# poyentung/ebsd-vae

Hardware: AMD Instinct MI355X
Metric: EBSD patterns/sec (128x128, fwd+bwd) (higher is better)
Workload: dtype fp32 I/O, f16x3 split MFMA; 1 GPU; c2: VariationalAutoEncoderRawData 128x128, latent 16, batch 256/GPU, fwd+loss+bwd+Adam; global_batch=256, image_size=128, latent_dim=16, parallelism=dp1

## Files before the change

### ebsd-vae_amd/csrc/conv_wgrad.hip

```cpp
#include <utility>

#include "common.h"
#include "../../include/ebsdvae.h"

namespace ev {

constexpr int WG_PT = 128;
constexpr int WG_AS = 48;

struct WgGeom {
  int TH, TW, NI, ntx, nty, tiles, slices, tps, lTW, ltpx;
};

static int wg_tw_pref() {
  static const int v = evh::env_int("EBSDVAE_WG_TW", 16, 8, 32);
  return (v == 8 || v == 32) ? v : 16;
}

static int wg_block_target(int pt) {
  static const int v = evh::env_int("EBSDVAE_WG_BLOCKS", 512, 64, 8192);
  return pt == 64 ? v : 1024;
}

static bool wg_geom(int B, int H, int W, int cin, int cout, WgGeom* g, int pt = WG_PT) {
// ... 14 lines not shown
  g->lTW = __builtin_ctz(g->TW);
  g->ltpx = __builtin_ctz(g->TH * g->TW);
  if ((1 << g->lTW) != g->TW || (1 << g->ltpx) != g->TH * g->TW) return false;
  g->nty = H / g->TH;
  const long imgs = (B + g->NI - 1) / g->NI;
  g->tiles = (int)(imgs * g->ntx * g->nty);
  const int co_t = cout == 1 ? 1 : (cout == 32 || g->TW == 8 ? cout / 32 : cout / 64);
  const int ci_t = cin == 1 ? 1 : (cout == 1 ? 1 : cin / 32);
  if (co_t <= 0 || ci_t <= 0) return false;
  const int want = wg_block_target(pt) / (co_t * ci_t);
  int tps = 4;
  while ((g->tiles + tps - 1) / tps > (want > 1 ? want : 1)) tps *= 2;
  g->tps = tps;
  g->slices = (g->tiles + tps - 1) / tps;
  return true;
}

static bool wg_pipe() {
  static const bool v = evh::env_flag("EBSDVAE_WG_PIPE", true);
  return v;
}
static int wg_pipe_cot(int cout) {
  static const bool wide = evh::env_flag("EBSDVAE_WG_CO128", true);
  return cout == 32 ? 32 : ((wide && cout % 128 == 0) ? 128 : 64);
}
static int wg_pipe_ci64_mode() {
  static const int v = evh::env_int("EBSDVAE_WG_CI64", 1, 0, 1);
  return v;
}
static int wg_pipe_cit(int cin, int cout) {
  if (wg_pipe_ci64_mode() == 0 || cout == 32 || cin % 64) return 32;
  return wg_pipe_cot(cout) == 64 ? 64 : 32;
}
static bool wg_pipe_geom(int B, int H, int W, int cin, int cout, WgGeom* g) {
  if (B <= 0 || H <= 0 || W <= 0 || cin <= 0 || cout <= 0) return false;
  if (H % 8 || W % 8 || cin % 32 || !(cout == 32 || cout % 64 == 0)) return false;
  if (((H / 8) & (H / 8 - 1)) || ((W / 8) & (W / 8 - 1))) return false;
  if (!ev_buf_bytes_ok(4LL * H * W * (cin > cout ? cin : cout) * 4)) return false;
  g->TW = 8; g->TH = 8; g->NI = 1;
  g->ntx = W / 8; g->nty = H / 8;
  g->lTW = 3; g->ltpx = 6;
  g->tiles = (int)((long)B * g->ntx * g->nty);
  const int cot = wg_pipe_cot(cout), cit = wg_pipe_cit(cin, cout);
  const int co_t = cout == 32 ? 1 : cout / cot;
  const bool eight = cot == 128 || cit == 64;
  const int want = wg_block_target(64) / (eight ? 2 : 1) / (co_t * (cin / cit));
  int tps = 4;
  while ((g->tiles + tps - 1) / tps > (want > 1 ? want : 1)) tps *= 2;
  g->tps = tps;
  g->slices = (g->tiles + tps - 1) / tps;
  return true;
}

static dim3 wg_pipe_grid(const WgGeom& g, int cin, int cout) {
  const int nm = (cout == 32 ? 1 : cout / wg_pipe_cot(cout)) * (cin / wg_pipe_cit(cin, cout));
  return dim3(8 * ((g.slices + 7) / 8) * nm);
}

EV_DEVINL void tile_origin(int t, const WgGeom& g, int& b0, int& y0, int& x0) {
  const int per_img = g.ntx * g.nty;
  const int ib = t / per_img, r = t - ib * per_img;
  b0 = ib * g.NI;
  y0 = (r / g.ntx) * g.TH;
  x0 = (r % g.ntx) * g.TW;
}

template <int TW>
struct WgTile {
  static constexpr int TH = TW == 32 ? 4 : 8;
  static constexpr int NI = TW == 8 ? 2 : 1;
  static constexpr int HP = TH + 2, WP = TW + 2;
  static constexpr int HALO = NI * HP * WP;
  static constexpr int IPX = TH * TW;
  static_assert(NI * IPX == WG_PT, "128-pixel tiles");
  static_assert(HALO * 8 <= 7 * 256, "7 halo float4 items per thread");
};

template <int NWCO, int KSPLIT, int MODE, int TW>
__global__ __launch_bounds__(256, 2) void wgrad_kernel(
    const float* __restrict__ src, const float2* __restrict__ sstats,
    const float* __restrict__ gy, float* __restrict__ wpart, float* __restrict__ bpart, int B,
    int H, int W, int Cin, int Cout, WgGeom g) {
  using T = WgTile<TW>;
  constexpr int CO_T = NWCO * 32;
  constexpr int GS = CO_T + 16;
  constexpr int QG = CO_T / 4;
  constexpr int KG = CO_T / 8;
  constexpr int KH = 7;
  constexpr bool NORM = (MODE == ACT_NORM || MODE == ACT_NORM_UP);
  constexpr bool UPS = (MODE == ACT_UP || MODE == ACT_NORM_UP);
  static_assert(NWCO * 2 * KSPLIT == 4, "4 waves per block");
  static_assert(MODE != ACT_NORM_POOL, "pool-fed layers use the materialised activation");
  constexpr int SPR = TW / (4 * KSPLIT);
  constexpr int ROW_UNROLL = 1;
  extern __shared__ __attribute__((aligned(16))) float smem[];
  float* lg = smem;
  float* la = smem + WG_PT * GS;
  const int tid = threadIdx.x, lane = tid & 63, wave = tid >> 6;
  const int wco = wave % NWCO, wci = (wave / NWCO) & 1, wk = wave / (2 * NWCO);
  const int slice = blockIdx.x, co0 = blockIdx.y * CO_T, ci0 = blockIdx.z * 32;
  const int l16 = lane & 15, kq = lane >> 4;
  const int Hs = UPS ? H / 2 : H, Ws = UPS ? W / 2 : W;
  const int qh = tid & 7;
  const int qg = tid % QG;
  const bool do_bias = blockIdx.z == 0;

  f32x4 acc[2][9];
#pragma unroll
  for (int f = 0; f < 2; ++f)
// ... 418 lines not shown
    for (int s = wk; s < KSTEPS; s += KSPLIT) {
      const int px0 = 32 * s + 4 * gq + q, px1 = px0 + 16;
      bf16x8w a[NPC][2];
#pragma unroll
      for (int i = 0; i < NPC; ++i)
#pragma unroll
        for (int f = 0; f < 2; ++f)
          a[i][f] = tr_frag(gimg + i * GY_PIECE + px0 * GSB + acol + f * 32,
                            gimg + i * GY_PIECE + px1 * GSB + acol + f * 32);
      int hp0, hp1;
      {
        const int im0 = px0 / T::IPX, rm0 = px0 % T::IPX;
        const int im1 = px1 / T::IPX, rm1 = px1 % T::IPX;
        hp0 = (im0 * T::HP + rm0 / TW) * T::WP + rm0 % TW;
        hp1 = (im1 * T::HP + rm1 / TW) * T::WP + rm1 % TW;
      }
      bf16x8w b[NPC];
#pragma unroll
      for (int tap = 0; tap < 9; ++tap) {
        const int toff = (tap / 3) * T::WP + tap % 3;
#pragma unroll
        for (int i = 0; i < NPC; ++i)
          b[i] = tr_frag(aimg + i * ACT_PIECE + (hp0 + toff) * WGS_ASB + bcol,
                         aimg + i * ACT_PIECE + (hp1 + toff) * WGS_ASB + bcol);
#pragma unroll
        for (int f = 0; f < 2; ++f) {
          f32x4 c = acc[f][tap];
          if constexpr (NP == 3) {
            c = __builtin_amdgcn_mfma_f32_16x16x32_bf16(a[1][f], b[1], c, 0, 0, 0);
            c = __builtin_amdgcn_mfma_f32_16x16x32_bf16(a[NP - 1][f], b[0], c, 0, 0, 0);
            c = __builtin_amdgcn_mfma_f32_16x16x32_bf16(a[0][f], b[NP - 1], c, 0, 0, 0);
          }
          c = mfma16_piece<NP>(a[1][f], b[0], c);
          c = mfma16_piece<NP>(a[0][f], b[1], c);
          c = mfma16_piece<NP>(a[0][f], b[0], c);
          acc[f][tap] = c;
        }
      }
    }
  }
  __syncthreads();
  wgrad_split_finish<NWCO, KSPLIT, F16>(acc, bs, wsm, wpart, bpart, slice, co0, ci0, Cin, Cout, gsc,
                                        do_bias);
}

template <class F, int... I>
EV_DEVINL void static_for_impl(F&& f, std::integer_sequence<int, I...>) {
  (f(std::integral_constant<int, I>()), ...);
}
template <int N, class F>
EV_DEVINL void static_for(F&& f) {
  static_for_impl(f, std::make_integer_sequence<int, N>());
}

template <int Q>
EV_DEVINL int wg_store_perm(int r) {
  if constexpr (Q == 8) return (r & ~3) | ((r >> 1) & 1) | ((r & 1) << 1);
  return r;
}

template <int NP, int NWCO, int KSPLIT, int MODE, int NWCI = 2, int FCO = 2>
__global__ __launch_bounds__(NWCO * NWCI * KSPLIT * 64, NWCO * NWCI * KSPLIT >= 8 ? 1 : 2) void wgrad_pipe_kernel(
    const float* __restrict__ src, const float2* __restrict__ sstats,
    const float* __restrict__ gy, float* __restrict__ wpart, float* __restrict__ bpart, int B,
    int H, int W, int Cin, int Cout, WgGeom g, const float* __restrict__ gmax, int gmT) {
  constexpr int TW = 8, PT = 64;
  using T = WgTileP<TW, PT>;
  constexpr int NPC = npc(NP);
  constexpr bool F16 = NP == NP_F16;
  constexpr int CO_T = NWCO * 16 * FCO;
  constexpr int CI_T = NWCI * 16;
  constexpr int GSB = CO_T * 2 + 32;
  constexpr int ASB = CI_T * 2 + 32;
  constexpr int QG = CO_T / 4;
  constexpr int QH = CI_T / 4;
  constexpr int NTH = NWCO * NWCI * KSPLIT * 64;
  constexpr int KG = PT * CO_T / 4 / NTH;
  constexpr int KH = (T::HALO * QH + NTH - 1) / NTH;
  constexpr int NIT = KG + KH;
  constexpr int KSTEPS = PT / 32;
  constexpr int NSLOT = (KSTEPS / KSPLIT) * 9;
  constexpr int GY_PIECE = PT * GSB;
  constexpr int ACT_PIECE = T::HALO * ASB;
  constexpr int BUF = NPC * (GY_PIECE + ACT_PIECE);
  constexpr bool NORM = (MODE == ACT_NORM || MODE == ACT_NORM_UP);
  constexpr bool UPS = (MODE == ACT_UP || MODE == ACT_NORM_UP);
  constexpr int kGyPol = CO_T <= 64 ? 2 : 0;
  static_assert(T::NI == 1 && T::HP == 10 && T::WP == 10, "8x8 tiles");
  static_assert(NWCO * NWCI * KSPLIT == 4 || NWCO * NWCI * KSPLIT == 8, "4 or 8 waves per block");
  static_assert((NWCI == 2 || NWCI == 4) && (FCO == 2 || FCO == 4), "wave / block tiles");
  static_assert(NTH % QG == 0 && NTH % QH == 0, "item channel groups fixed per thread");
  static_assert(KSTEPS % KSPLIT == 0 && NIT <= NSLOT, "item slots");
  static_assert(MODE != ACT_NORM_POOL, "pool-fed layers use the materialised activation");
  extern __shared__ __attribute__((aligned(16))) char wsm[];
  const int tid = threadIdx.x, lane = tid & 63, wave = tid >> 6;
  const int wco = wave % NWCO, wci = (wave / NWCO) % NWCI, wk = wave / (NWCI * NWCO);
  const int nco = Cout / CO_T, nm = nco * (Cin / CI_T);
  const int xcd = blockIdx.x & 7, wq = blockIdx.x >> 3, m = wq % nm;
  const int slice = (wq / nm) * 8 + xcd;
  if (slice >= g.slices) return;
  const int co0 = (m % nco) * CO_T, ci0 = (m / nco) * CI_T;
  const int Hs = UPS ? H / 2 : H, Ws = UPS ? W / 2 : W;
  const int qh = tid % QH, qg = tid % QG;

  f32x4 acc[FCO][9];
#pragma unroll
  for (int f = 0; f < FCO; ++f)
#pragma unroll
    for (int t = 0; t < 9; ++t) acc[f][t] = f32x4{0.f, 0.f, 0.f, 0.f};
  double bs[4] = {0.0, 0.0, 0.0, 0.0};

  const int per_img = g.ntx * g.nty;
  const int t_beg = slice * g.tps;
  const int t_end = min(t_beg + g.tps, g.tiles);
  int gshift = 0;
  if constexpr (F16)
    if (t_beg < t_end) gshift = f16_gshift(gmax, gmT, t_beg / per_img, (t_end - 1) / per_img);
  const float gsc = ldexpf(1.f, gshift);

  int gyo[KG], glo[KG];
#pragma unroll
  for (int k = 0; k < KG; ++k) {
    const int px = wg_store_perm<QG>((tid + NTH * k) / QG), r = px / TW, c = px % TW;
    gyo[k] = (r * W + c) * Cout + co0 + qg * 4;
    glo[k] = px * GSB + qg * 8;
  }
  int hdr[KH], hdc[KH], hlo[KH];
  int hbo[KH];
  const int srow = Ws * Cin * 4;
#pragma unroll
  for (int k = 0; k < KH; ++k) {
    const int pix = wg_store_perm<QH>((tid + NTH * k) / QH);
    hdr[k] = pix < T::HALO ? pix / T::WP - 1 : -(1 << 20);
    hdc[k] = pix % T::WP - 1;
    hlo[k] = pix * ASB + qh * 8;
    hbo[k] = pix < T::HALO ? (UPS ? (hdr[k] >> 1) * srow + (hdc[k] >> 1) * Cin * 4
                                  : hdr[k] * srow + hdc[k] * Cin * 4) + (ci0 + qh * 4) * 4
                           : (int)0x80000000;
  }
  const int gimg_bytes = H * W * Cout * 4, simg_bytes = Hs * Ws * Cin * 4;

  float4 rg[KG], rh[KH];
  float2 st_l[4], st_s[4];
  int lb = 0, ly = 0, lx = 0;
  int sb = 0, sy = 0, sx = 0;
  const int lgx = 31 - __builtin_clz(g.ntx), lgp = lgx + 31 - __builtin_clz(g.nty);
  auto tile_at = [&](int t, int& b0, int& y0, int& x0) EV_LAMBDA_INLINE {
    const int rr = t & ((1 << lgp) - 1);
    b0 = t >> lgp; y0 = (rr >> lgx) * T::TH; x0 = (rr & (g.ntx - 1)) * TW;
  };
  __amdgpu_buffer_rsrc_t rgy, rsrc;
  int gtoff = 0, stoff = 0;
  auto set_tile = [&]() EV_LAMBDA_INLINE {
    rgy = __builtin_amdgcn_make_buffer_rsrc((void*)(gy + (size_t)lb * H * W * Cout), 0, gimg_bytes,
                                            0x00020000);
    rsrc = __builtin_amdgcn_make_buffer_rsrc((void*)(src + (size_t)lb * Hs * Ws * Cin), 0,
                                             simg_bytes, 0x00020000);
    gtoff = (ly * W + lx) * Cout * 4;
    stoff = UPS ? (ly >> 1) * srow + (lx >> 1) * Cin * 4 : ly * srow + lx * Cin * 4;
  };
  auto load_stats = [&]() EV_LAMBDA_INLINE {
    set_tile();
    if constexpr (NORM) {
      const float2* sp = sstats + (size_t)lb * Cin + ci0 + qh * 4;
      st_l[0] = norm_fs(sp[0]); st_l[1] = norm_fs(sp[1]); st_l[2] = norm_fs(sp[2]); st_l[3] = norm_fs(sp[3]);
    }
  };
  auto in_img = [&](int k, int y0, int x0) EV_LAMBDA_INLINE {
    return (unsigned)(y0 + hdr[k]) < (unsigned)H && (unsigned)(x0 + hdc[k]) < (unsigned)W;
  };
  auto issue_item = [&](auto j_c) EV_LAMBDA_INLINE {
    constexpr int j = decltype(j_c)::value;
    if constexpr (j < KG) {
      rg[j] = __builtin_bit_cast(float4, __builtin_amdgcn_raw_buffer_load_b128(
                                             rgy, gtoff + gyo[j] * 4, 0, kGyPol));
    } else {
      constexpr int k = j - KG;
      rh[k] = __builtin_bit_cast(float4, __builtin_amdgcn_raw_buffer_load_b128(
                                             rsrc, stoff + hbo[k], 0, 0));
    }
  };
  float4 tb;
  auto store_item = [&](auto j_c, char* buf) EV_LAMBDA_INLINE {
    constexpr int j = decltype(j_c)::value;
    if constexpr (j < KG) {
      float4 v = rg[j];
      tb.x += v.x; tb.y += v.y; tb.z += v.z; tb.w += v.w;
      if constexpr (F16) v = make_float4(v.x * gsc, v.y * gsc, v.z * gsc, v.w * gsc);
      store_pieces<NP>(buf + glo[j], GY_PIECE, v);
    } else {
      constexpr int k = j - KG;
      if (hdr[k] > -2) {
        float4 v = make_float4(0.f, 0.f, 0.f, 0.f);
        if (in_img(k, sy, sx)) {
          v = rh[k];
          if (NORM)
            v = make_float4(normact_fs(v.x, st_s[0]), normact_fs(v.y, st_s[1]),
                            normact_fs(v.z, st_s[2]), normact_fs(v.w, st_s[3]));
        }
        store_pieces<NP>(buf + NPC * GY_PIECE + hlo[k], ACT_PIECE, v);
      }
    }
  };
  auto all_items = [&](auto fn) EV_LAMBDA_INLINE { static_for<NIT>(fn); };
  auto shift = [&]() EV_LAMBDA_INLINE {
    sb = lb; sy = ly; sx = lx;
#pragma unroll
    for (int i = 0; i < 4; ++i) st_s[i] = st_l[i];
  };

  const int gq = lane >> 4, i16 = lane & 15, q = i16 >> 2, p4 = i16 & 3;
  const int acol = (wco * 16 * FCO + 4 * p4) * 2;
  const int bcol = (wci * 16 + 4 * p4) * 2;

  if (t_beg < t_end) {
    tile_at(t_beg, lb, ly, lx);
    load_stats();
    all_items([&](auto j) EV_LAMBDA_INLINE { issue_item(j); });
    shift();
    tb = make_float4(0.f, 0.f, 0.f, 0.f);
    all_items([&](auto j) EV_LAMBDA_INLINE { store_item(j, wsm); });
    bs[0] += (double)tb.x; bs[1] += (double)tb.y; bs[2] += (double)tb.z; bs[3] += (double)tb.w;
    tile_at(min(t_beg + 1, t_end - 1), lb, ly, lx);
    load_stats();
    all_items([&](auto j) EV_LAMBDA_INLINE { issue_item(j); });
  }
  __syncthreads();
  for (int t = t_beg; t < t_end; ++t) {
    const int cur = (t - t_beg) & 1;
    const char* gimg = wsm + cur * BUF;
    const char* aimg = gimg + NPC * GY_PIECE;
    char* nbuf = wsm + (1 - cur) * BUF;
    shift();
    tile_at(min(t + 2, t_end - 1), lb, ly, lx);
    load_stats();
    tb = make_float4(0.f, 0.f, 0.f, 0.f);
    static_for<KSTEPS / KSPLIT>([&](auto si_c) EV_LAMBDA_INLINE {
      constexpr int si = decltype(si_c)::value;
      const int s = wk + si * KSPLIT;
      const int px0 = 32 * s + 4 * gq + q, px1 = px0 + 16;
      bf16x8w a[NPC][FCO];
#pragma unroll
      for (int i = 0; i < NPC; ++i)
#pragma unroll
        for (int f = 0; f < FCO; ++f)
          a[i][f] = tr_frag(gimg + i * GY_PIECE + px0 * GSB + acol + f * 32,
                            gimg + i * GY_PIECE + px1 * GSB + acol + f * 32);
      const int hp0 = (px0 / TW) * T::WP + px0 % TW, hp1 = (px1 / TW) * T::WP + px1 % TW;
      static_for<9>([&](auto tap_c) EV_LAMBDA_INLINE {
        constexpr int tap = decltype(tap_c)::value;
        constexpr int toff = (tap / 3) * T::WP + tap % 3;
        bf16x8w b[NPC];
#pragma unroll
        for (int i = 0; i < NPC; ++i)
          b[i] = tr_frag(aimg + i * ACT_PIECE + (hp0 + toff) * ASB + bcol,
                         aimg + i * ACT_PIECE + (hp1 + toff) * ASB + bcol);
#pragma unroll
        for (int f = 0; f < FCO; ++f) {
          f32x4 c = acc[f][tap];
          c = mfma16_piece<NP>(a[1][f], b[0], c);
          c = mfma16_piece<NP>(a[0][f], b[1], c);
          c = mfma16_piece<NP>(a[0][f], b[0], c);
          acc[f][tap] = c;
        }
        all_items([&](auto j_c) EV_LAMBDA_INLINE {
          constexpr int j = decltype(j_c)::value;
          if constexpr (si * 9 + tap == (j * NSLOT) / NIT) {
            store_item(j_c, nbuf);
            issue_item(j_c);
          }
        });
      });
    });
    if (t + 1 < t_end) {
      bs[0] += (double)tb.x; bs[1] += (double)tb.y; bs[2] += (double)tb.z; bs[3] += (double)tb.w;
    }
    __syncthreads();
  }
  wgrad_split_finish<NWCO, KSPLIT, F16, FCO, NWCI>(acc, bs, wsm, wpart, bpart, slice, co0, ci0, Cin,
                                                   Cout, gsc, ci0 == 0);
}

__global__ __launch_bounds__(128) void wgrad_cin1_kernel(
    const float* __restrict__ src, const float2* __restrict__ sstats, int smode,
    const float* __restrict__ gy, float* __restrict__ wpart, float* __restrict__ bpart, int B,
    int H, int W, int Cout, WgGeom g) {
  constexpr int GS = 48;
  extern __shared__ __attribute__((aligned(16))) float smem[];
  float* lg = smem;
  float* la = smem + WG_PT * GS;
  const int tid = threadIdx.x, lane = tid & 63, wave = tid >> 6;
  const int slice = blockIdx.x;
  const int HP = g.TH + 2, WP = g.TW + 2, halo = g.NI * HP * WP;
  const int l16 = lane & 15, kq = lane >> 4;
  const int tapj = l16 < 9 ? l16 : 0;
  const int tkh = tapj / 3, tkw = tapj % 3;
  f32x4 acc = f32x4{0.f, 0.f, 0.f, 0.f};
  double bsum = 0.0;
  const int t_beg = slice * g.tps, t_end = min(t_beg + g.tps, g.tiles);
  const int tpx = g.TH * g.TW;
  for (int t = t_beg; t < t_end; ++t) {
    int b0, y0, x0;
    tile_origin(t, g, b0, y0, x0);
    __syncthreads();
    for (int i = tid; i < WG_PT * 8; i += 128) {
      const int px = i >> 3, q = i & 7;
      const int img = px >> g.ltpx, rem = px & (tpx - 1);
      const int r = rem >> g.lTW, c = rem & (g.TW - 1);
      const int gb = b0 + img;
// ... 229 lines not shown
    once = true;
  }
  hipLaunchKernelGGL(k, grid, dim3(256), lds, s, src, (const float2*)st, gy, wpart, bpart, B, H, W,
                     cin, cout, g);
}

template <int NWCO, int KSPLIT, int MODE>
static void launch_wg(dim3 grid, size_t lds, hipStream_t s, const float* src, const float* st,
                      const float* gy, float* wpart, float* bpart, int B, int H, int W, int cin,
                      int cout, const WgGeom& g) {
  if (g.TW == 32)
    launch_wg_tw<NWCO, KSPLIT, MODE, 32>(grid, lds, s, src, st, gy, wpart, bpart, B, H, W, cin, cout, g);
  else if (g.TW == 16)
    launch_wg_tw<NWCO, KSPLIT, MODE, 16>(grid, lds, s, src, st, gy, wpart, bpart, B, H, W, cin, cout, g);
  else if constexpr (NWCO == 1)
    launch_wg_tw<NWCO, KSPLIT, MODE, 8>(grid, lds, s, src, st, gy, wpart, bpart, B, H, W, cin, cout, g);
}

template <int NP, int NWCO, int KSPLIT, int MODE, int TW, int PT>
static void launch_wgs_tw(dim3 grid, hipStream_t s, const float* src, const float* st,
                          const float* gy, float* wpart, float* bpart, int B, int H, int W, int cin,
                          int cout, const WgGeom& g, const float* gmax, int gmT) {
  using T = WgTileP<TW, PT>;
  constexpr int CO_T = NWCO * 32;
  const size_t lds_img = (size_t)npc(NP) * ((size_t)PT * (CO_T * 2 + 32) + (size_t)T::HALO * WGS_ASB);
  const size_t lds_fold = KSPLIT == 2 ? (size_t)2 * 72 * 64 * 4 : 0;
  const size_t lds_bias = 256 * 4 * 8;
  size_t lds = lds_img;
  if (lds < lds_fold) lds = lds_fold;
  if (lds < lds_bias) lds = lds_bias;
  auto k = wgrad_split_kernel<NP, NWCO, KSPLIT, MODE, TW, PT>;
  static bool once = false;
  if (!once) {
    (void)hipFuncSetAttribute((const void*)k, hipFuncAttributeMaxDynamicSharedMemorySize, 160 * 1024);
    once = true;
  }
  hipLaunchKernelGGL(k, grid, dim3(256), lds, s, src, (const float2*)st, gy, wpart, bpart, B, H, W,
                     cin, cout, g, gmax, gmT);
}

template <int NP, int NWCO, int KSPLIT, int MODE>
static void launch_wgs(dim3 grid, hipStream_t s, const float* src, const float* st, const float* gy,
                       float* wpart, float* bpart, int B, int H, int W, int cin, int cout,
                       const WgGeom& g, const float* gmax, int gmT) {
  constexpr int PT = 64;
  if (g.TW == 32)
    launch_wgs_tw<NP, NWCO, KSPLIT, MODE, 32, PT>(grid, s, src, st, gy, wpart, bpart, B, H, W, cin, cout, g, gmax, gmT);
  else if (g.TW == 16)
    launch_wgs_tw<NP, NWCO, KSPLIT, MODE, 16, PT>(grid, s, src, st, gy, wpart, bpart, B, H, W, cin, cout, g, gmax, gmT);
  else if constexpr (NWCO == 1)
    launch_wgs_tw<NP, NWCO, KSPLIT, MODE, 8, PT>(grid, s, src, st, gy, wpart, bpart, B, H, W, cin, cout, g, gmax, gmT);
}

template <int NP, int NWCO, int KSPLIT, int MODE, int NWCI = 2, int FCO = 2>
static void launch_wgp(dim3 grid, hipStream_t s, const float* src, const float* st, const float* gy,
                       float* wpart, float* bpart, int B, int H, int W, int cin, int cout,
                       const WgGeom& g, const float* gmax, int gmT) {
  constexpr int CO_T = NWCO * 16 * FCO, CI_T = NWCI * 16;
  constexpr int NTH = NWCO * NWCI * KSPLIT * 64;
  const size_t lds_img = 2 * (size_t)npc(NP) * ((size_t)64 * (CO_T * 2 + 32) + (size_t)100 * (CI_T * 2 + 32));
  const size_t lds_fold = KSPLIT == 2 ? (size_t)NWCO * NWCI * FCO * 36 * 64 * 4 : 0;
  size_t lds = lds_img;
  if (lds < lds_fold) lds = lds_fold;
  if (lds < (size_t)NTH * 4 * 8) lds = (size_t)NTH * 4 * 8;
  auto k = wgrad_pipe_kernel<NP, NWCO, KSPLIT, MODE, NWCI, FCO>;
  static bool once = false;
  if (!once) {
    (void)hipFuncSetAttribute((const void*)k, hipFuncAttributeMaxDynamicSharedMemorySize, 160 * 1024);
    once = true;
  }
  hipLaunchKernelGGL(k, grid, dim3(NTH), lds, s, src, (const float2*)st, gy, wpart, bpart, B, H, W,
                     cin, cout, g, gmax, gmT);
}

template <class F>
static void with_src_mode(int mode, F&& f) {
  evh::with_const<ACT_RAW, ACT_NORM, ACT_UP, ACT_NORM_UP>(mode, f);
}
template <int N> using Int = std::integral_constant<int, N>;

template <int NP>
static void dispatch_wgp(int mode, bool narrow, dim3 grid, hipStream_t s, const float* src,
                         const float* st, const float* gy, float* wpart, float* bpart, int B, int H,
                         int W, int cin, int cout, const WgGeom& g, const float* gmax, int gmT) {
  with_src_mode(mode, [&](auto m) {
    auto go = [&](auto nwco, auto ksplit, auto nwci) {
      launch_wgp<NP, decltype(nwco)::value, decltype(ksplit)::value, decltype(m)::value,
                 decltype(nwci)::value>(grid, s, src, st, gy, wpart, bpart, B, H, W, cin, cout, g, gmax, gmT);
    };
    if (narrow) go(Int<1>(), Int<2>(), Int<2>());
    else if (wg_pipe_cit(cin, cout) == 64) go(Int<2>(), Int<1>(), Int<4>());
    else if (wg_pipe_cot(cout) == 128) go(Int<4>(), Int<1>(), Int<2>());
    else go(Int<2>(), Int<1>(), Int<2>());
  });
}

template <int NP>
static void dispatch_wgs(int mode, bool narrow, dim3 grid, hipStream_t s, const float* src,
                         const float* st, const float* gy, float* wpart, float* bpart, int B, int H,
                         int W, int cin, int cout, const WgGeom& g, const float* gmax, int gmT) {
  with_src_mode(mode, [&](auto m) {
    constexpr int M = decltype(m)::value;
    if (narrow) launch_wgs<NP, 1, 2, M>(grid, s, src, st, gy, wpart, bpart, B, H, W, cin, cout, g, gmax, gmT);
    else launch_wgs<NP, 2, 1, M>(grid, s, src, st, gy, wpart, bpart, B, H, W, cin, cout, g, gmax, gmT);
  });
}

static bool wgs_geom_ok(const WgGeom& g, int pt) {
  if (pt == 128)
    return (g.TW == 32 && g.TH == 4) || (g.TW == 16 && g.TH == 8 && g.NI == 1) ||
           (g.TW == 8 && g.TH == 8 && g.NI == 2);
  return (g.TW == 32 && g.TH == 2) || (g.TW == 16 && g.TH == 4 && g.NI == 1) ||
         (g.TW == 8 && g.TH == 8 && g.NI == 1);
}

}

using namespace ev;

extern "C" int ebsdvae_conv3x3_wgrad_split_slices(int B, int H, int W, int cin, int cout, int pieces) {
  WgGeom g;
  if (pieces != 2 && pieces != 3 && pieces != NP_F16) return -1;
  if (B <= 0 || H <= 0 || W <= 0 || cin <= 0 || cout <= 0) return -1;
  if (cin % 32 || !(cout == 32 || cout % 64 == 0)) return -1;
  if (pieces != 3 && wg_pipe()) return wg_pipe_geom(B, H, W, cin, cout, &g) ? g.slices : -1;
  const int pt = 64;
  if (!wg_geom(B, H, W, cin, cout, &g, pt) || !wgs_geom_ok(g, pt)) return -1;
  return g.slices;
}

extern "C" int ebsdvae_conv3x3_wgrad_split(const float* src, const float* src_stats, int src_mode,
                                           const float* gy, float* wpart, float* bpart, int B,
                                           int H, int W, int cin, int cout, int pieces,
                                           ebsdvae_stream_t stream) {
  WgGeom g;
  EV_REQUIRE(src && gy && wpart && bpart && B > 0, "conv3x3_wgrad_split: null pointer");
  EV_REQUIRE(pieces == 2 || pieces == 3, "conv3x3_wgrad_split: pieces=%d (2 or 3)", pieces);
  EV_REQUIRE(src_mode >= 0 && src_mode <= 4 && src_mode != ACT_NORM_POOL,
             "conv3x3_wgrad_split: bad src_mode %d (pool-fed layers pass the pooled activation RAW)",
             src_mode);
  EV_REQUIRE(src_mode == ACT_RAW || src_mode == ACT_UP || src_stats, "conv3x3_wgrad_split: NORM needs stats");
  EV_REQUIRE(cin % 32 == 0 && (cout == 32 || cout % 64 == 0), "conv3x3_wgrad_split: cin=%d cout=%d unsupported",
             cin, cout);
  hipStream_t s = (hipStream_t)stream;
  if (pieces == 2 && wg_pipe()) {
    EV_REQUIRE(wg_pipe_geom(B, H, W, cin, cout, &g), "conv3x3_wgrad_split: unsupported shape H=%d W=%d", H, W);
    const bool narrow = cout == 32;
    dispatch_wgp<2>(src_mode, narrow, wg_pipe_grid(g, cin, cout), s, src, src_stats, gy, wpart, bpart, B,
                    H, W, cin, cout, g, nullptr, 0);
    return evh::check_launch("wgrad_split");
  }
  const int pt = 64;
  EV_REQUIRE(wg_geom(B, H, W, cin, cout, &g, pt) && wgs_geom_ok(g, pt),
             "conv3x3_wgrad_split: unsupported shape H=%d W=%d", H, W);
  const bool narrow = cout == 32 || g.TW == 8 || (pieces == 3 && g.TW == 16);
  const dim3 grid(g.slices, narrow ? cout / 32 : cout / 64, cin / 32);
  if (pieces == 3)
    dispatch_wgs<3>(src_mode, narrow, grid, s, src, src_stats, gy, wpart, bpart, B, H, W, cin, cout, g,
                    nullptr, 0);
  else
    dispatch_wgs<2>(src_mode, narrow, grid, s, src, src_stats, gy, wpart, bpart, B, H, W, cin, cout, g,
                    nullptr, 0);
  return evh::check_launch("wgrad_split");
}

extern "C" int ebsdvae_conv3x3_wgrad_f16(const float* src, const float* src_stats, int src_mode,
                                         const float* gy, const float* gmax, int gm_tiles,
                                         float* wpart, float* bpart, int B, int H, int W, int cin,
                                         int cout, ebsdvae_stream_t stream) {
  WgGeom g;
  EV_REQUIRE(src && gy && gmax && gm_tiles > 0 && wpart && bpart && B > 0,
             "conv3x3_wgrad_f16: null pointer or no gradient maxima");
  EV_REQUIRE(src_mode >= 0 && src_mode <= 4 && src_mode != ACT_NORM_POOL,
             "conv3x3_wgrad_f16: bad src_mode %d (pool-fed layers pass the pooled activation RAW)",
             src_mode);
  EV_REQUIRE(src_mode == ACT_RAW || src_mode == ACT_UP || src_stats, "conv3x3_wgrad_f16: NORM needs stats");
  EV_REQUIRE(cin % 32 == 0 && (cout == 32 || cout % 64 == 0), "conv3x3_wgrad_f16: cin=%d cout=%d unsupported",
             cin, cout);
  if (wg_pipe()) {
    EV_REQUIRE(wg_pipe_geom(B, H, W, cin, cout, &g), "conv3x3_wgrad_f16: unsupported shape H=%d W=%d", H, W);
    const bool narrow = cout == 32;
    dispatch_wgp<NP_F16>(src_mode, narrow, wg_pipe_grid(g, cin, cout), (hipStream_t)stream, src, src_stats,
                         gy, wpart, bpart, B, H, W, cin, cout, g, gmax, gm_tiles);
    return evh::check_launch("wgrad_f16");
  }
  const int pt = 64;
  EV_REQUIRE(wg_geom(B, H, W, cin, cout, &g, pt) && wgs_geom_ok(g, pt),
             "conv3x3_wgrad_f16: unsupported shape H=%d W=%d", H, W);
  const bool narrow = cout == 32 || g.TW == 8;
  const dim3 grid(g.slices, narrow ? cout / 32 : cout / 64, cin / 32);
  dispatch_wgs<NP_F16>(src_mode, narrow, grid, (hipStream_t)stream, src, src_stats, gy, wpart, bpart,
                       B, H, W, cin, cout, g, gmax, gm_tiles);
  return evh::check_launch("wgrad_f16");
}

extern "C" int ebsdvae_conv3x3_wgrad_slices(int B, int H, int W, int cin, int cout) {
  WgGeom g;
  if (!wg_geom(B, H, W, cin, cout, &g)) return -1;
  return g.slices;
}

extern "C" int ebsdvae_conv3x3_wgrad(const float* src, const float* src_stats, int src_mode,
                                     const float* gy, float* wpart, float* bpart, int B, int H,
                                     int W, int cin, int cout, ebsdvae_stream_t stream) {
  WgGeom g;
  EV_REQUIRE(src && gy && wpart && bpart && B > 0, "conv3x3_wgrad: null pointer");
  EV_REQUIRE(src_mode >= 0 && src_mode <= 4, "conv3x3_wgrad: bad src_mode");
  EV_REQUIRE(src_mode == ACT_RAW || src_mode == ACT_UP || src_stats, "conv3x3_wgrad: NORM needs stats");
  EV_REQUIRE(wg_geom(B, H, W, cin, cout, &g), "conv3x3_wgrad: unsupported shape H=%d W=%d", H, W);
  hipStream_t s = (hipStream_t)stream;
  if (cin == 1) {
    EV_REQUIRE(cout == 32, "conv3x3_wgrad: cin=1 needs cout=32");
    hipLaunchKernelGGL(wgrad_cin1_kernel, dim3(g.slices), dim3(128), wg_lds(1, g, 32), s, src,
                       (const float2*)src_stats, src_mode, gy, wpart, bpart, B, H, W, cout, g);
    return evh::check_launch("wgrad_cin1");
  }
  if (cout == 1) {
    EV_REQUIRE(cin == 32, "conv3x3_wgrad: cout=1 needs cin=32");
    hipLaunchKernelGGL(wgrad_cout1_kernel, dim3(g.slices), dim3(128), wg_lds(2, g, 0), s, src,
                       (const float2*)src_stats, src_mode, gy, wpart, bpart, B, H, W, cin, g);
    return evh::check_launch("wgrad_cout1");
  }
  EV_REQUIRE(cin % 32 == 0 && (cout == 32 || cout % 64 == 0), "conv3x3_wgrad: cin=%d cout=%d unsupported",
             cin, cout);
  EV_REQUIRE((g.TW == 32 && g.TH == 4) || (g.TW == 16 && g.TH == 8 && g.NI == 1) ||
                 (g.TW == 8 && g.TH == 8 && g.NI == 2),
             "conv3x3_wgrad: unsupported tile geometry H=%d W=%d", H, W);
  EV_REQUIRE(src_mode != ACT_NORM_POOL,
             "conv3x3_wgrad: pass the pooled activation materialised by the forward (RAW)");
  const bool narrow = cout == 32 || g.TW == 8;
  const size_t lds = wg_lds(0, g, narrow ? 32 : 64);
  const dim3 grid(g.slices, cout / (narrow ? 32 : 64), cin / 32);
  with_src_mode(src_mode, [&](auto m) {
    constexpr int M = decltype(m)::value;
    if (narrow) launch_wg<1, 2, M>(grid, lds, s, src, src_stats, gy, wpart, bpart, B, H, W, cin, cout, g);
    else launch_wg<2, 1, M>(grid, lds, s, src, src_stats, gy, wpart, bpart, B, H, W, cin, cout, g);
// ... 78 lines not shown
```

Before: 30450 patterns/s.

## Add parity-decomposed and source-resolution-halo wgrad paths for upsample-fed convs

Adds two new variants of the pipelined weight-gradient kernel for layers fed by a nearest-neighbour upsample. The parity path (off by default) splits output pixels into four parity classes so each correlates against the low-resolution source with 2x2 effective taps, then folds them into the 3x3 weights. The source-halo path (on by default) stages only a 6x6 source-resolution halo instead of the 10x10 upsampled one and remaps the tap addresses. Both aim to cut halo loads and LDS traffic, at the cost of more template instances and more complex indexing.

```diff
diff --git a/ebsd-vae_amd/csrc/conv_wgrad.hip b/ebsd-vae_amd/csrc/conv_wgrad.hip
--- a/ebsd-vae_amd/csrc/conv_wgrad.hip
+++ b/ebsd-vae_amd/csrc/conv_wgrad.hip
@@ -90,9 +90,34 @@
   return true;
 }
 
+static bool wg_upphase() {
+  static const bool v = evh::env_flag("EBSDVAE_WG_UPPHASE", false);
+  return v;
+}
+static bool wg_srchalo() {
+  static const bool v = evh::env_flag("EBSDVAE_WG_SRCHALO", true);
+  return v;
+}
+static int wg_upp_shape(int mode, int H, int W, int cin, int cout) {
+  if (!wg_upphase() || !(mode == ACT_UP || mode == ACT_NORM_UP) || H % 16 || W % 16) return 0;
+  if (cout == 32) return 1;
+  return (wg_pipe_ci64_mode() != 0 && cin % 64 == 0 && cout % 64 == 0) ? 2 : 0;
+}
+static bool wg_pipe_geom_upp(int shape, int B, int H, int W, int cin, int cout, WgGeom* g) {
+  if (!shape || H % 16 || W % 16 || !wg_pipe_geom(B, H, W, cin, cout, g)) return false;
+  const int nm = shape == 1 ? cin / 32 : (cout / 64) * (cin / 64);
+  const int want = wg_block_target(64) / (shape == 2 ? 2 : 1) / nm;
+  g->ntx = W / 16; g->nty = H / 16;
+  g->tiles = (int)((long)B * g->ntx * g->nty);
+  int tps = 1;
+  while ((g->tiles + tps - 1) / tps > (want > 1 ? want : 1)) tps *= 2;
+  g->tps = tps;
+  return g->slices == (g->tiles + tps - 1) / tps;
+}
+
+static dim3 wg_pipe_grid(const WgGeom& g, int nm) { return dim3(8 * ((g.slices + 7) / 8) * nm); }
 static dim3 wg_pipe_grid(const WgGeom& g, int cin, int cout) {
-  const int nm = (cout == 32 ? 1 : cout / wg_pipe_cot(cout)) * (cin / wg_pipe_cit(cin, cout));
-  return dim3(8 * ((g.slices + 7) / 8) * nm);
+  return wg_pipe_grid(g, (cout == 32 ? 1 : cout / wg_pipe_cot(cout)) * (cin / wg_pipe_cit(cin, cout)));
 }
 
 EV_DEVINL void tile_origin(int t, const WgGeom& g, int& b0, int& y0, int& x0) {
@@ -617,6 +642,7 @@
 EV_DEVINL void static_for(F&& f) {
   static_for_impl(f, std::make_integer_sequence<int, N>());
 }
+template <int N> using Int = std::integral_constant<int, N>;
 
 template <int Q>
 EV_DEVINL int wg_store_perm(int r) {
@@ -624,7 +650,11 @@
   return r;
 }
 
-template <int NP, int NWCO, int KSPLIT, int MODE, int NWCI = 2, int FCO = 2>
+#ifndef EV_WG_UP_GD
+#define EV_WG_UP_GD 1
+#endif
+template <int NP, int NWCO, int KSPLIT, int MODE, int NWCI = 2, int FCO = 2, bool UPP = false,
+          bool SH = false>
 __global__ __launch_bounds__(NWCO * NWCI * KSPLIT * 64, NWCO * NWCI * KSPLIT >= 8 ? 1 : 2) void wgrad_pipe_kernel(
     const float* __restrict__ src, const float2* __restrict__ sstats,
     const float* __restrict__ gy, float* __restrict__ wpart, float* __restrict__ bpart, int B,
@@ -641,7 +671,9 @@
   constexpr int QH = CI_T / 4;
   constexpr int NTH = NWCO * NWCI * KSPLIT * 64;
   constexpr int KG = PT * CO_T / 4 / NTH;
-  constexpr int KH = (T::HALO * QH + NTH - 1) / NTH;
+  constexpr int HWP = SH ? 6 : T::WP;
+  constexpr int HALO_N = SH ? 36 : T::HALO;
+  constexpr int KH = (HALO_N * QH + NTH - 1) / NTH;
   constexpr int NIT = KG + KH;
   constexpr int KSTEPS = PT / 32;
   constexpr int NSLOT = (KSTEPS / KSPLIT) * 9;
@@ -657,6 +689,8 @@
   static_assert(NTH % QG == 0 && NTH % QH == 0, "item channel groups fixed per thread");
   static_assert(KSTEPS % KSPLIT == 0 && NIT <= NSLOT, "item slots");
   static_assert(MODE != ACT_NORM_POOL, "pool-fed layers use the materialised activation");
+  static_assert(!UPP || (UPS && FCO == 2 && KH <= 4), "parity steps: upsample-fed, 16 x FCO accumulators");
+  static_assert(!SH || (UPS && !UPP), "source-resolution halo: upsample-fed, full-resolution steps");
   extern __shared__ __attribute__((aligned(16))) char wsm[];
   const int tid = threadIdx.x, lane = tid & 63, wave = tid >> 6;
   const int wco = wave % NWCO, wci = (wave / NWCO) % NWCI, wk = wave / (NWCI * NWCO);
@@ -669,10 +703,12 @@
   const int qh = tid % QH, qg = tid % QG;
 
   f32x4 acc[FCO][9];
-#pragma unroll
-  for (int f = 0; f < FCO; ++f)
-#pragma unroll
-    for (int t = 0; t < 9; ++t) acc[f][t] = f32x4{0.f, 0.f, 0.f, 0.f};
+  if constexpr (!UPP) {
+#pragma unroll
+    for (int f = 0; f < FCO; ++f)
+#pragma unroll
+      for (int t = 0; t < 9; ++t) acc[f][t] = f32x4{0.f, 0.f, 0.f, 0.f};
+  }
   double bs[4] = {0.0, 0.0, 0.0, 0.0};
 
   const int per_img = g.ntx * g.nty;
@@ -687,7 +723,7 @@
 #pragma unroll
   for (int k = 0; k < KG; ++k) {
     const int px = wg_store_perm<QG>((tid + NTH * k) / QG), r = px / TW, c = px % TW;
-    gyo[k] = (r * W + c) * Cout + co0 + qg * 4;
+    gyo[k] = (UPP ? 2 * (r * W + c) : r * W + c) * Cout + co0 + qg * 4;
     glo[k] = px * GSB + qg * 8;
   }
   int hdr[KH], hdc[KH], hlo[KH];
@@ -696,10 +732,10 @@
 #pragma unroll
   for (int k = 0; k < KH; ++k) {
     const int pix = wg_store_perm<QH>((tid + NTH * k) / QH);
-    hdr[k] = pix < T::HALO ? pix / T::WP - 1 : -(1 << 20);
-    hdc[k] = pix % T::WP - 1;
+    hdr[k] = pix < HALO_N ? pix / HWP - 1 : -(1 << 20);
+    hdc[k] = pix % HWP - 1;
     hlo[k] = pix * ASB + qh * 8;
-    hbo[k] = pix < T::HALO ? (UPS ? (hdr[k] >> 1) * srow + (hdc[k] >> 1) * Cin * 4
+    hbo[k] = pix < HALO_N ? (UPS && !UPP && !SH ? (hdr[k] >> 1) * srow + (hdc[k] >> 1) * Cin * 4
                                   : hdr[k] * srow + hdc[k] * Cin * 4) + (ci0 + qh * 4) * 4
                            : (int)0x80000000;
   }
@@ -717,12 +753,13 @@
   __amdgpu_buffer_rsrc_t rgy, rsrc;
   int gtoff = 0, stoff = 0;
   auto set_tile = [&]() EV_LAMBDA_INLINE {
-    rgy = __builtin_amdgcn_make_buffer_rsrc((void*)(gy + (size_t)lb * H * W * Cout), 0, gimg_bytes,
-                                            0x00020000);
+    if constexpr (!UPP)
+      rgy = __builtin_amdgcn_make_buffer_rsrc((void*)(gy + (size_t)lb * H * W * Cout), 0, gimg_bytes,
+                                              0x00020000);
     rsrc = __builtin_amdgcn_make_buffer_rsrc((void*)(src + (size_t)lb * Hs * Ws * Cin), 0,
                                              simg_bytes, 0x00020000);
     gtoff = (ly * W + lx) * Cout * 4;
-    stoff = UPS ? (ly >> 1) * srow + (lx >> 1) * Cin * 4 : ly * srow + lx * Cin * 4;
+    stoff = UPS && !UPP ? (ly >> 1) * srow + (lx >> 1) * Cin * 4 : ly * srow + lx * Cin * 4;
   };
   auto load_stats = [&]() EV_LAMBDA_INLINE {
     set_tile();
@@ -732,7 +769,10 @@
     }
   };
   auto in_img = [&](int k, int y0, int x0) EV_LAMBDA_INLINE {
-    return (unsigned)(y0 + hdr[k]) < (unsigned)H && (unsigned)(x0 + hdc[k]) < (unsigned)W;
+    if constexpr (SH)
+      return (unsigned)((y0 >> 1) + hdr[k]) < (unsigned)Hs && (unsigned)((x0 >> 1) + hdc[k]) < (unsigned)Ws;
+    return (unsigned)(y0 + hdr[k]) < (unsigned)(UPP ? Hs : H) &&
+           (unsigned)(x0 + hdc[k]) < (unsigned)(UPP ? Ws : W);
   };
   auto issue_item = [&](auto j_c) EV_LAMBDA_INLINE {
     constexpr int j = decltype(j_c)::value;
@@ -778,6 +818,195 @@
   const int acol = (wco * 16 * FCO + 4 * p4) * 2;
   const int bcol = (wci * 16 + 4 * p4) * 2;
 
+  if constexpr (UPP) {
+    constexpr int GD = EV_WG_UP_GD;
+    static_assert(GD == 1 || GD == 2, "gy prefetch depth");
+    constexpr int NSL = (KSTEPS / KSPLIT) * 4;
+    constexpr int HSTEP = 4 / KH >= 1 ? 4 / KH : 1;
+    static_assert(KG + 1 <= NSL, "item slots of a parity step");
+    f32x4 pacc[FCO][16];
+#pragma unroll
+    for (int f = 0; f < FCO; ++f)
+#pragma unroll
+      for (int t = 0; t < 16; ++t) pacc[f][t] = f32x4{0.f, 0.f, 0.f, 0.f};
+    float4 rq[GD][KG];
+    __amdgpu_buffer_rsrc_t rgy_c, rgy_s;
+    int gt_c = 0, gt_s = 0;
+    int pof[4];
+#pragma unroll
+    for (int par = 0; par < 4; ++par) pof[par] = ((par >> 1) * W + (par & 1)) * Cout * 4;
+    auto gy_tile = [&](int b0, int y0, int x0, __amdgpu_buffer_rsrc_t& r, int& off) EV_LAMBDA_INLINE {
+      r = __builtin_amdgcn_make_buffer_rsrc((void*)(gy + (size_t)b0 * H * W * Cout), 0, gimg_bytes,
+                                            0x00020000);
+      off = (2 * y0 * W + 2 * x0) * Cout * 4;
+    };
+    constexpr int GROWS = NTH / QG / TW;
+    static_assert(GROWS * TW * QG == NTH && (NTH / QG) % 4 == 0, "gy items whole tile rows apart");
+    const int gyv = gyo[0] * 4, glv = glo[0];
+    const int gstep = GROWS * 2 * W * Cout * 4;
+    int hpk[KH];
+#pragma unroll
+    for (int k = 0; k < KH; ++k) {
+      const int pix = wg_store_perm<QH>((tid + NTH * k) / QH);
+      hpk[k] = pix < T::HALO ? ((pix / T::WP) << 16) | (pix % T::WP) : (0x7fff << 16);
+    }
+    const int hcv = (ci0 + qh * 4) * 4;
+    auto issue_gy = [&](auto v_c, auto j_c) EV_LAMBDA_INLINE {
+      constexpr int v = decltype(v_c)::value, j = decltype(j_c)::value;
+      rq[v & (GD - 1)][j] = __builtin_bit_cast(
+          float4, __builtin_amdgcn_raw_buffer_load_b128(v >= 4 ? rgy_s : rgy_c, gyv,
+                                                        (v >= 4 ? gt_s : gt_c) + pof[v & 3] + j * gstep,
+                                                        kGyPol));
+    };
+    auto store_gy = [&](auto v_c, auto j_c, char* buf) EV_LAMBDA_INLINE {
+      constexpr int v = decltype(v_c)::value, j = decltype(j_c)::value;
+      float4 w = rq[v & (GD - 1)][j];
+      tb.x += w.x; tb.y += w.y; tb.z += w.z; tb.w += w.w;
+      if constexpr (F16) w = make_float4(w.x * gsc, w.y * gsc, w.z * gsc, w.w * gsc);
+      store_pieces<NP>(buf + glv + j * (NTH / QG) * GSB, GY_PIECE, w);
+    };
+    auto issue_h = [&](auto k_c) EV_LAMBDA_INLINE {
+      constexpr int k = decltype(k_c)::value;
+      const int hr = (hpk[k] >> 16) - 1, hc = (hpk[k] & 0xffff) - 1;
+      const int vo = hr < T::HP ? stoff + hr * srow + hc * Cin * 4 + hcv : (int)0x80000000;
+      rh[k] = __builtin_bit_cast(float4, __builtin_amdgcn_raw_buffer_load_b128(rsrc, vo, 0, 0));
+    };
+    auto store_h = [&](auto k_c, char* buf) EV_LAMBDA_INLINE {
+      constexpr int k = decltype(k_c)::value;
+      const int hr = hpk[k] >> 16, hc = hpk[k] & 0xffff;
+      if (hr < T::HP) {
+        float4 v = make_float4(0.f, 0.f, 0.f, 0.f);
+        if ((unsigned)(sy + hr - 1) < (unsigned)Hs && (unsigned)(sx + hc - 1) < (unsigned)Ws) {
+          v = rh[k];
+          if (NORM)
+            v = make_float4(normact_fs(v.x, st_s[0]), normact_fs(v.y, st_s[1]),
+                            normact_fs(v.z, st_s[2]), normact_fs(v.w, st_s[3]));
+        }
+        store_pieces<NP>(buf + NPC * GY_PIECE + (hr * T::WP + hc) * ASB + qh * 8, ACT_PIECE, v);
+      }
+    };
+    auto stage_tile = [&]() EV_LAMBDA_INLINE {
+      sb = lb; sy = ly; sx = lx;
+      if constexpr (NORM) {
+        const float2* sp = sstats + (size_t)sb * Cin + ci0 + qh * 4;
+        st_s[0] = norm_fs(sp[0]); st_s[1] = norm_fs(sp[1]); st_s[2] = norm_fs(sp[2]); st_s[3] = norm_fs(sp[3]);
+      }
+    };
+    if (t_beg < t_end) {
+      tile_at(t_beg, lb, ly, lx);
+      set_tile();
+      gy_tile(lb, ly, lx, rgy_s, gt_s);
+      rgy_c = rgy_s; gt_c = gt_s;
+      static_for<KH>([&](auto k) EV_LAMBDA_INLINE { issue_h(k); });
+      static_for<KG>([&](auto j) EV_LAMBDA_INLINE { issue_gy(Int<0>(), j); });
+      stage_tile();
+      tb = make_float4(0.f, 0.f, 0.f, 0.f);
+      static_for<KG>([&](auto j) EV_LAMBDA_INLINE { store_gy(Int<0>(), j, wsm); });
+      static_for<KH>([&](auto k) EV_LAMBDA_INLINE { store_h(k, wsm); });
+      bs[0] += (double)tb.x; bs[1] += (double)tb.y; bs[2] += (double)tb.z; bs[3] += (double)tb.w;
+      tile_at(min(t_beg + 1, t_end - 1), lb, ly, lx);
+      set_tile();
+      static_for<KH>([&](auto k) EV_LAMBDA_INLINE { issue_h(k); });
+      static_for<GD>([&](auto d) EV_LAMBDA_INLINE {
+        static_for<KG>([&](auto j) EV_LAMBDA_INLINE { issue_gy(Int<1 + decltype(d)::value>(), j); });
+      });
+    }
+    __syncthreads();
+    for (int t = t_beg; t < t_end; ++t) {
+      const int aset = (t - t_beg) & 1;
+      const char* aimg = wsm + aset * BUF + NPC * GY_PIECE;
+      char* anext = wsm + (1 - aset) * BUF;
+#pragma unroll
+      for (int k = 0; k < KH; ++k) asm volatile("" : "+v"(hpk[k]));
+      rgy_c = rgy_s; gt_c = gt_s;
+      stage_tile();
+      gy_tile(sb, sy, sx, rgy_s, gt_s);
+      tile_at(min(t + 2, t_end - 1), lb, ly, lx);
+      set_tile();
+      static_for<4>([&](auto par_c) EV_LAMBDA_INLINE {
+        constexpr int par = decltype(par_c)::value, py = par >> 1, px = par & 1;
+        constexpr int hk = par / HSTEP;
+        constexpr bool has_h = par % HSTEP == 0 && hk < KH;
+        constexpr int NITP = KG + (has_h ? 1 : 0);
+        const char* gimg = wsm + (par & 1) * BUF;
+        char* gnext = wsm + ((par + 1) & 1) * BUF;
+        tb = make_float4(0.f, 0.f, 0.f, 0.f);
+        static_for<KSTEPS / KSPLIT>([&](auto si_c) EV_LAMBDA_INLINE {
+          constexpr int si = decltype(si_c)::value;
+          const int s = wk + si * KSPLIT;
+          const int px0 = 32 * s + 4 * gq + q, px1 = px0 + 16;
+          bf16x8w a[NPC][FCO];
+#pragma unroll
+          for (int i = 0; i < NPC; ++i)
+#pragma unroll
+            for (int f = 0; f < FCO; ++f)
+              a[i][f] = tr_frag(gimg + i * GY_PIECE + px0 * GSB + acol + f * 32,
+                                gimg + i * GY_PIECE + px1 * GSB + acol + f * 32);
+          const int hp0 = (px0 / TW) * T::WP + px0 % TW, hp1 = (px1 / TW) * T::WP + px1 % TW;
+          static_for<4>([&](auto tt_c) EV_LAMBDA_INLINE {
+            constexpr int tt = decltype(tt_c)::value;
+            constexpr int toff = (py + (tt >> 1)) * T::WP + px + (tt & 1);
+            bf16x8w b[NPC];
+#pragma unroll
+            for (int i = 0; i < NPC; ++i)
+              b[i] = tr_frag(aimg + i * ACT_PIECE + (hp0 + toff) * ASB + bcol,
+                             aimg + i * ACT_PIECE + (hp1 + toff) * ASB + bcol);
+#pragma unroll
+            for (int f = 0; f < FCO; ++f) {
+              f32x4 c = pacc[f][par * 4 + tt];
+              c = mfma16_piece<NP>(a[1][f], b[0], c);
+              c = mfma16_piece<NP>(a[0][f], b[1], c);
+              c = mfma16_piece<NP>(a[0][f], b[0], c);
+              pacc[f][par * 4 + tt] = c;
+            }
+            static_for<KG>([&](auto j_c) EV_LAMBDA_INLINE {
+              constexpr int j = decltype(j_c)::value;
+              if constexpr (si * 4 + tt == (j * NSL) / NITP) {
+                store_gy(Int<par + 1>(), j_c, gnext);
+                issue_gy(Int<par + 1 + GD>(), j_c);
+              }
+            });
+            if constexpr (has_h && si * 4 + tt == (KG * NSL) / NITP) {
+              store_h(Int<hk>(), anext);
+              issue_h(Int<hk>());
+            }
+          });
+        });
+        if (par < 3 || t + 1 < t_end) {
+          bs[0] += (double)tb.x; bs[1] += (double)tb.y; bs[2] += (double)tb.z; bs[3] += (double)tb.w;
+        }
+        __syncthreads();
+      });
+    }
+#pragma unroll
+    for (int f = 0; f < FCO; ++f)
+#pragma unroll
+      for (int tap = 0; tap < 9; ++tap) {
+        const int ky = tap / 3, kx = tap % 3;
+        f32x4 c = f32x4{0.f, 0.f, 0.f, 0.f};
+#pragma unroll
+        for (int par = 0; par < 4; ++par) {
+          const int py = par >> 1, px = par & 1;
+          const int ay = py == 0 ? (ky >= 1) : (ky == 2), ax = px == 0 ? (kx >= 1) : (kx == 2);
+          c += pacc[f][par * 4 + ay * 2 + ax];
+        }
+        acc[f][tap] = c;
+      }
+    wgrad_split_finish<NWCO, KSPLIT, F16, FCO, NWCI>(acc, bs, wsm, wpart, bpart, slice, co0, ci0, Cin,
+                                                     Cout, gsc, ci0 == 0);
+    return;
+  }
+
+  int sh_ry[3], sh_cx[3];
+  if constexpr (SH) {
+    const int pxw = 32 * wk + 4 * gq + q, r = pxw / TW, c = pxw % TW;
+#pragma unroll
+    for (int d = 0; d < 3; ++d) {
+      sh_ry[d] = (((r + d - 1) >> 1) + 1) * HWP * ASB + bcol;
+      sh_cx[d] = (((c + d - 1) >> 1) + 1) * ASB;
+    }
+  }
+
   if (t_beg < t_end) {
     tile_at(t_beg, lb, ly, lx);
     load_stats();
@@ -816,10 +1045,17 @@
         constexpr int tap = decltype(tap_c)::value;
         constexpr int toff = (tap / 3) * T::WP + tap % 3;
         bf16x8w b[NPC];
-#pragma unroll
-        for (int i = 0; i < NPC; ++i)
-          b[i] = tr_frag(aimg + i * ACT_PIECE + (hp0 + toff) * ASB + bcol,
-                         aimg + i * ACT_PIECE + (hp1 + toff) * ASB + bcol);
+        if constexpr (SH) {
+          const char* r0 = aimg + sh_ry[tap / 3] + sh_cx[tap % 3] + si * KSPLIT * 2 * HWP * ASB;
+#pragma unroll
+          for (int i = 0; i < NPC; ++i)
+            b[i] = tr_frag(r0 + i * ACT_PIECE, r0 + i * ACT_PIECE + HWP * ASB);
+        } else {
+#pragma unroll
+          for (int i = 0; i < NPC; ++i)
+            b[i] = tr_frag(aimg + i * ACT_PIECE + (hp0 + toff) * ASB + bcol,
+                           aimg + i * ACT_PIECE + (hp1 + toff) * ASB + bcol);
+        }
 #pragma unroll
         for (int f = 0; f < FCO; ++f) {
           f32x4 c = acc[f][tap];
@@ -1155,7 +1391,8 @@
     launch_wgs_tw<NP, NWCO, KSPLIT, MODE, 8, PT>(grid, s, src, st, gy, wpart, bpart, B, H, W, cin, cout, g, gmax, gmT);
 }
 
-template <int NP, int NWCO, int KSPLIT, int MODE, int NWCI = 2, int FCO = 2>
+template <int NP, int NWCO, int KSPLIT, int MODE, int NWCI = 2, int FCO = 2, bool UPP = false,
+          bool SH = false>
 static void launch_wgp(dim3 grid, hipStream_t s, const float* src, const float* st, const float* gy,
                        float* wpart, float* bpart, int B, int H, int W, int cin, int cout,
                        const WgGeom& g, const float* gmax, int gmT) {
@@ -1166,7 +1403,7 @@
   size_t lds = lds_img;
   if (lds < lds_fold) lds = lds_fold;
   if (lds < (size_t)NTH * 4 * 8) lds = (size_t)NTH * 4 * 8;
-  auto k = wgrad_pipe_kernel<NP, NWCO, KSPLIT, MODE, NWCI, FCO>;
+  auto k = wgrad_pipe_kernel<NP, NWCO, KSPLIT, MODE, NWCI, FCO, UPP, SH>;
   static bool once = false;
   if (!once) {
     (void)hipFuncSetAttribute((const void*)k, hipFuncAttributeMaxDynamicSharedMemorySize, 160 * 1024);
@@ -1180,15 +1417,22 @@
 static void with_src_mode(int mode, F&& f) {
   evh::with_const<ACT_RAW, ACT_NORM, ACT_UP, ACT_NORM_UP>(mode, f);
 }
-template <int N> using Int = std::integral_constant<int, N>;
 
 template <int NP>
 static void dispatch_wgp(int mode, bool narrow, dim3 grid, hipStream_t s, const float* src,
                          const float* st, const float* gy, float* wpart, float* bpart, int B, int H,
                          int W, int cin, int cout, const WgGeom& g, const float* gmax, int gmT) {
   with_src_mode(mode, [&](auto m) {
+    constexpr int M = decltype(m)::value;
     auto go = [&](auto nwco, auto ksplit, auto nwci) {
-      launch_wgp<NP, decltype(nwco)::value, decltype(ksplit)::value, decltype(m)::value,
+      if constexpr (M == ACT_UP || M == ACT_NORM_UP) {
+        if (wg_srchalo()) {
+          launch_wgp<NP, decltype(nwco)::value, decltype(ksplit)::value, M, decltype(nwci)::value, 2,
+                     false, true>(grid, s, src, st, gy, wpart, bpart, B, H, W, cin, cout, g, gmax, gmT);
+          return;
+        }
+      }
+      launch_wgp<NP, decltype(nwco)::value, decltype(ksplit)::value, M,
                  decltype(nwci)::value>(grid, s, src, st, gy, wpart, bpart, B, H, W, cin, cout, g, gmax, gmT);
     };
     if (narrow) go(Int<1>(), Int<2>(), Int<2>());
@@ -1196,6 +1440,29 @@
     else if (wg_pipe_cot(cout) == 128) go(Int<4>(), Int<1>(), Int<2>());
     else go(Int<2>(), Int<1>(), Int<2>());
   });
+}
+
+template <int NP>
+static bool run_wgp(int mode, hipStream_t s, const float* src, const float* st, const float* gy,
+                    float* wpart, float* bpart, int B, int H, int W, int cin, int cout,
+                    const float* gmax, int gmT) {
+  WgGeom g;
+  const int shape = wg_upp_shape(mode, H, W, cin, cout);
+  if (wg_pipe_geom_upp(shape, B, H, W, cin, cout, &g)) {
+    const dim3 grid = wg_pipe_grid(g, shape == 1 ? cin / 32 : (cout / 64) * (cin / 64));
+    evh::with_const<ACT_UP, ACT_NORM_UP>(mode, [&](auto m) {
+      constexpr int M = decltype(m)::value;
+      if (shape == 1)
+        launch_wgp<NP, 1, 2, M, 2, 2, true>(grid, s, src, st, gy, wpart, bpart, B, H, W, cin, cout, g, gmax, gmT);
+      else
+        launch_wgp<NP, 2, 1, M, 4, 2, true>(grid, s, src, st, gy, wpart, bpart, B, H, W, cin, cout, g, gmax, gmT);
+    });
+    return true;
+  }
+  if (!wg_pipe_geom(B, H, W, cin, cout, &g)) return false;
+  dispatch_wgp<NP>(mode, cout == 32, wg_pipe_grid(g, cin, cout), s, src, st, gy, wpart, bpart, B, H, W,
+                   cin, cout, g, gmax, gmT);
+  return true;
 }
 
 template <int NP>
@@ -1247,10 +1514,8 @@
              cin, cout);
   hipStream_t s = (hipStream_t)stream;
   if (pieces == 2 && wg_pipe()) {
-    EV_REQUIRE(wg_pipe_geom(B, H, W, cin, cout, &g), "conv3x3_wgrad_split: unsupported shape H=%d W=%d", H, W);
-    const bool narrow = cout == 32;
-    dispatch_wgp<2>(src_mode, narrow, wg_pipe_grid(g, cin, cout), s, src, src_stats, gy, wpart, bpart, B,
-                    H, W, cin, cout, g, nullptr, 0);
+    EV_REQUIRE(run_wgp<2>(src_mode, s, src, src_stats, gy, wpart, bpart, B, H, W, cin, cout, nullptr, 0),
+               "conv3x3_wgrad_split: unsupported shape H=%d W=%d", H, W);
     return evh::check_launch("wgrad_split");
   }
   const int pt = 64;
@@ -1281,10 +1546,9 @@
   EV_REQUIRE(cin % 32 == 0 && (cout == 32 || cout % 64 == 0), "conv3x3_wgrad_f16: cin=%d cout=%d unsupported",
              cin, cout);
   if (wg_pipe()) {
-    EV_REQUIRE(wg_pipe_geom(B, H, W, cin, cout, &g), "conv3x3_wgrad_f16: unsupported shape H=%d W=%d", H, W);
-    const bool narrow = cout == 32;
-    dispatch_wgp<NP_F16>(src_mode, narrow, wg_pipe_grid(g, cin, cout), (hipStream_t)stream, src, src_stats,
-                         gy, wpart, bpart, B, H, W, cin, cout, g, gmax, gm_tiles);
+    EV_REQUIRE(run_wgp<NP_F16>(src_mode, (hipStream_t)stream, src, src_stats, gy, wpart, bpart, B, H, W,
+                               cin, cout, gmax, gm_tiles),
+               "conv3x3_wgrad_f16: unsupported shape H=%d W=%d", H, W);
     return evh::check_launch("wgrad_f16");
   }
   const int pt = 64;
```

Result: no change. 30620 patterns/s (median of 6 runs) (+0.6%).
